# jpinedev/OpenCL-Raytracer

Hardware: AMD Instinct MI355X
Metric: Mrays/s (primary+reflect+shadow) at 4096x4096, 1/2/4/8 GPU; max RGB diff vs ref (higher is better)
Workload: dtype f32

## Files before the change

opencl-raytracer_amd/csrc/rt_device.h:

```cpp
#pragma once

#include <hip/hip_runtime.h>
#include <stdint.h>

namespace rt {

constexpr float kMaxFloat = 3.402823466e+38F;

struct HotObject {
    float4 row0;
    float4 row1;
    float4 row2;
    uint32_t type;
    uint32_t pad[3];
};
struct ColdObject {
    float4 mv_row[4];
    float4 inv_row3;
    float4 amb_absorb;
    float4 dif_shine;
    float4 spec_type;
};
struct ObjectRecord {
    float4 inv_row[3];
// ... 351 lines not shown
    uint32_t line = (p + kWarmAhead) * 2u + (__lane_id() & 63u);
    const uint32_t last = n_pairs * 2u - 1u;
    line = line < last ? line : last;
    w.pending = *reinterpret_cast<const uint32_t*>(reinterpret_cast<const char*>(pairs) + (uint64_t)line * 64u);
}
__device__ __forceinline__ void l2_warm_finish(Warm& w) {
    asm volatile("" ::"v"(w.sink ^ w.pending));
}

template <int AM, bool DW0>
__device__ __forceinline__ void closest_hit(const HotPair* __restrict__ pairs, uint32_t n_pairs, const Ray& ray, float& T,
                                            int& index) {
    if (n_pairs == 0) return;
    const RaySplat r = splat(ray);
    Warm warm;
    HotPair a = pairs[0];
    uint32_t p = 0;
    for (; p + 1 < n_pairs; p += 2) {
        if ((p & (kWarmPeriod - 1u)) == 0u) l2_warm(pairs, n_pairs, p, warm);
        const HotPair b = pairs[p + 1];
        closest_pair<AM, DW0>(a, (int)p, r, T, index);
        a = pairs[(p + 2 < n_pairs) ? p + 2 : p + 1];
        closest_pair<AM, DW0>(b, (int)p + 1, r, T, index);
    }
    if (p < n_pairs) closest_pair<AM, DW0>(a, (int)p, r, T, index);
    l2_warm_finish(warm);
}

template <int AM>
__device__ __forceinline__ bool occludes(uint32_t type, float sx, float sy, float sz, float dx, float dy, float dz) {
    float t;
    bool cand = false;
    if (type == 0u) cand = sphere_candidate<AM>(sx, sy, sz, dx, dy, dz, t);
    else if (type == 1u) cand = box_candidate<AM>(sx, sy, sz, dx, dy, dz, t);
    return cand && !(t >= 1.f);
}

template <int AM>
__device__ __forceinline__ bool any_hit_pair(const HotPair& h, const RaySplat& r) {
    f2 sx, sy, sz, dx, dy, dz;
    pair_object_space<AM, true>(h, r, sx, sy, sz, dx, dy, dz);
    bool occ = false;
    if ((h.type_a | h.type_b) == 0u) {
        const f2 rad = pair_radical<AM>(sx, sy, sz, dx, dy, dz);
        const bool ca = !(rad.x < 0), cb = !(rad.y < 0);
        if (ca || cb) {
            if (ca) occ = occludes<AM>(0u, sx.x, sy.x, sz.x, dx.x, dy.x, dz.x);
            if (cb && !occ) occ = occludes<AM>(0u, sx.y, sy.y, sz.y, dx.y, dy.y, dz.y);
        }
    } else {
        occ = occludes<AM>(h.type_a, sx.x, sy.x, sz.x, dx.x, dy.x, dz.x);
        if (!occ) occ = occludes<AM>(h.type_b, sx.y, sy.y, sz.y, dx.y, dy.y, dz.y);
    }
    return occ;
}

template <int AM>
__device__ __forceinline__ bool any_hit_before_one(const HotPair* __restrict__ pairs, uint32_t n_pairs, const Ray& ray,
                                                   uint32_t* pairs_visited = nullptr) {
    if (pairs_visited) *pairs_visited = 0;
    if (n_pairs == 0) return false;
    const RaySplat r = splat(ray);
    bool occluded = false, done = false;
    Warm warm;
    HotPair a = pairs[0];
    uint32_t p = 0;
    for (; p + 1 < n_pairs; p += 2) {
        if ((p & (kWarmPeriod - 1u)) == 0u) l2_warm(pairs, n_pairs, p, warm);
        const HotPair b = pairs[p + 1];
        occluded |= any_hit_pair<AM>(a, r);
        a = pairs[(p + 2 < n_pairs) ? p + 2 : p + 1];
        occluded |= any_hit_pair<AM>(b, r);
        if (__ballot(!occluded) == 0ull) { done = true; p += 2; break; }
    }
    if (!done && p < n_pairs) {
        if (__ballot(!occluded) != 0ull) { occluded |= any_hit_pair<AM>(a, r); p = n_pairs; }
    }
    if (pairs_visited) *pairs_visited = p;
    l2_warm_finish(warm);
    return occluded;
}

template <int AM, bool DW0>
__device__ __forceinline__ void object_space_one(const RT_CONST HotObjectC* o, const Ray& ray, float& sx, float& sy,
                                                 float& sz, float& dx, float& dy, float& dz) {
    const f4 r0 = o->row0, r1 = o->row1, r2 = o->row2;
    sx = row4<AM>(r0.x, r0.y, r0.z, r0.w, ray.sx, ray.sy, ray.sz, ray.sw);
    sy = row4<AM>(r1.x, r1.y, r1.z, r1.w, ray.sx, ray.sy, ray.sz, ray.sw);
    sz = row4<AM>(r2.x, r2.y, r2.z, r2.w, ray.sx, ray.sy, ray.sz, ray.sw);
    if constexpr (DW0) {
        dx = row3<AM>(r0.x, r0.y, r0.z, ray.dx, ray.dy, ray.dz);
        dy = row3<AM>(r1.x, r1.y, r1.z, ray.dx, ray.dy, ray.dz);
        dz = row3<AM>(r2.x, r2.y, r2.z, ray.dx, ray.dy, ray.dz);
    } else {
        dx = row4<AM>(r0.x, r0.y, r0.z, r0.w, ray.dx, ray.dy, ray.dz, ray.dw);
        dy = row4<AM>(r1.x, r1.y, r1.z, r1.w, ray.dx, ray.dy, ray.dz, ray.dw);
        dz = row4<AM>(r2.x, r2.y, r2.z, r2.w, ray.dx, ray.dy, ray.dz, ray.dw);
    }
}

template <int AM, bool DW0>
__device__ __forceinline__ void closest_hit_small(const HotObject* __restrict__ hot_, uint32_t n, bool use_mask, uint64_t mask,
                                                  const Ray& ray, float& T, int& index) {
    const RT_CONST HotObjectC* hot = (const RT_CONST HotObjectC*)(hot_);
    if (use_mask) {
        while (mask) {
            const int k = __builtin_ctzll(mask);
            mask &= mask - 1ull;
            float sx, sy, sz, dx, dy, dz;
            object_space_one<AM, DW0>(hot + k, ray, sx, sy, sz, dx, dy, dz);
            closest_update<AM>(hot[k].type, sx, sy, sz, dx, dy, dz, k, T, index);
        }
    } else {
        for (uint32_t k = 0; k < n; ++k) {
            float sx, sy, sz, dx, dy, dz;
            object_space_one<AM, DW0>(hot + k, ray, sx, sy, sz, dx, dy, dz);
            closest_update<AM>(hot[k].type, sx, sy, sz, dx, dy, dz, (int)k, T, index);
        }
    }
}

template <int AM>
__device__ __forceinline__ bool any_hit_small(const HotObject* __restrict__ hot_, uint32_t n, const Ray& ray) {
    const RT_CONST HotObjectC* hot = (const RT_CONST HotObjectC*)(hot_);
    bool occluded = false;
    for (uint32_t k = 0; k < n; ++k) {
        float sx, sy, sz, dx, dy, dz;
        object_space_one<AM, true>(hot + k, ray, sx, sy, sz, dx, dy, dz);
        occluded |= occludes<AM>(hot[k].type, sx, sy, sz, dx, dy, dz);
        if (__ballot(!occluded) == 0ull) break;
    }
    return occluded;
}

struct ObjRows {
    float4 r0, r1, r2;
    uint32_t type, pad0;
};

template <int AM>
__device__ __forceinline__ void materialise(const ObjectRecord* __restrict__ objrec, const ColdObject* __restrict__ cold,
                                            int index, float t, const Ray& ray, HitRec& h, bool affine = false, ObjRows* rows = nullptr,
                                            float* absorption = nullptr) {
    const ObjectRecord* o = objrec + index;
    const ColdObject* c = cold + index;
    const uint32_t type = o->type;
    if (rows) { rows->r0 = o->inv_row[0]; rows->r1 = o->inv_row[1]; rows->r2 = o->inv_row[2]; rows->type = type; rows->pad0 = o->pad0; }
    if (absorption) *absorption = o->absorption;
    if (type == 2u) {
        const float4 e1 = o->inv_row[1], e2 = o->inv_row[2];
        h.px = fma_<AM>(t, ray.dx, ray.sx);
        h.py = fma_<AM>(t, ray.dy, ray.sy);
        h.pz = fma_<AM>(t, ray.dz, ray.sz);
        h.pw = fma_<AM>(t, ray.dw, ray.sw);
        float nx = e1.y * e2.z - e1.z * e2.y;
        float ny = e1.z * e2.x - e1.x * e2.z;
        float nz = e1.x * e2.y - e1.y * e2.x;
        normalize3(nx, ny, nz);
        h.nx = nx; h.ny = ny; h.nz = nz;
        const float k2 = dot3(ray.dx, ray.dy, ray.dz, nx, ny, nz) * -2.0f;
        h.rx = fma_<AM>(k2, nx, ray.dx);
        h.ry = fma_<AM>(k2, ny, ray.dy);
        h.rz = fma_<AM>(k2, nz, ray.dz);
        h.index = index;
        return;
    }
    const float4 r0 = o->inv_row[0], r1 = o->inv_row[1], r2 = o->inv_row[2];
    const float sx = row4<AM>(r0.x, r0.y, r0.z, r0.w, ray.sx, ray.sy, ray.sz, ray.sw);
    const float sy = row4<AM>(r1.x, r1.y, r1.z, r1.w, ray.sx, ray.sy, ray.sz, ray.sw);
    const float sz = row4<AM>(r2.x, r2.y, r2.z, r2.w, ray.sx, ray.sy, ray.sz, ray.sw);
    const float dx = row4<AM>(r0.x, r0.y, r0.z, r0.w, ray.dx, ray.dy, ray.dz, ray.dw);
    const float dy = row4<AM>(r1.x, r1.y, r1.z, r1.w, ray.dx, ray.dy, ray.dz, ray.dw);
    const float dz = row4<AM>(r2.x, r2.y, r2.z, r2.w, ray.dx, ray.dy, ray.dz, ray.dw);
    float sw, dw;
    if (affine) {
        sw = ray.sw;
        dw = ray.dw;
    } else {
        const float4 r3 = c->inv_row3;
        sw = row4<AM>(r3.x, r3.y, r3.z, r3.w, ray.sx, ray.sy, ray.sz, ray.sw);
        dw = row4<AM>(r3.x, r3.y, r3.z, r3.w, ray.dx, ray.dy, ray.dz, ray.dw);
// ... 272 lines not shown
```

opencl-raytracer_amd/csrc/rt_wavefront.hip:

```cpp
#include "rt_kernels.h"
#include "rt_grid.h"

#include <algorithm>
#include <cstdio>
#include <cstdlib>
#include <cstring>

namespace rt {

enum : uint32_t {
    F_SX, F_SY, F_SZ, F_SW, F_DX, F_DY, F_DZ, F_DW,
    F_A0, F_A1, F_A2, F_A3, F_A4, F_A5, F_A6, F_A7,
    F_PX, F_PY, F_PZ, F_HIDX,
    F_NX, F_NY, F_NZ, F_PHASE,
    F_ABR, F_ABG, F_ABB, F_AP,
    F_RES_T, F_RES_I, F_RES_ANY, F_BOUNCES,
    F_RX, F_RY, F_RZ, F_PW,
    F_RR, F_RG, F_RB, F_SPARE,
    F_AR, F_AG, F_AB, F_DR, F_DG, F_DB, F_SR, F_SG,
    F_SB, F_CR, F_CG, F_CB,
    F_COUNT
};
static_assert(F_COUNT % 4 == 0 && F_PX == 16, "blocks of four after the two ray records");
enum : uint32_t { PH_DONE = 0, PH_PRIMARY = 1, PH_SHADOW_PRIMARY = 2, PH_SHADOW_REFLECT = 3, PH_REFLECT = 4 };
constexpr uint32_t PH_FLAG_REFLECTION_SENT = 0x100u;
constexpr uint32_t PH_FLAG_REFLECTION_PENDING = 0x200u;
constexpr uint32_t kPhaseLightShift = 10;
static_assert(kPhaseLightShift == 10, "rt_create limits the light count to 2^22 - 1");

enum : uint32_t {
    RS_NEXT_CLOSEST = 0, RS_NEXT_ANY = 1,
    RS_SLICE_A = 2, RS_SLICE_B = 3,
    RS_N_CLOSEST = 4, RS_N_ANY = 5,
    RS_CUR = 6,
    RS_FINISH = 7,
    RS_ROUNDS = 8,
    RS_NEXT_SINGLES = 10,
    RS_N_SINGLES = 11,
    RS_WORDS = 16
};

struct WfParams {
    RenderParams rp;
    float* st;
    uint32_t* qs[2][2];
    uint32_t* q_closest;
    uint32_t* q_any;
    uint32_t* q_prev_closest;
    uint32_t* q_prev_any;
    uint32_t* counts;
    const HotPair* shadow_pairs;
    GridDesc grid;
    ScreenTiles tiles;
    LightTiles ltiles;
    BlockGrid bgrid;
    uint32_t n_prev_closest, n_prev_any;
    int kernel;
    uint32_t first_round;
    uint32_t identity_queue;
    uint32_t count_rays;
};

__device__ __forceinline__ bool resolve_round(WfParams& w) {
    const uint32_t* rs = w.counts;
    const bool odd = (rs[RS_CUR] & 1u) != 0u;
    w.q_prev_closest = odd ? w.qs[1][0] : w.qs[0][0];
    w.q_prev_any = odd ? w.qs[1][1] : w.qs[0][1];
    w.q_closest = odd ? w.qs[0][0] : w.qs[1][0];
    w.q_any = odd ? w.qs[0][1] : w.qs[1][1];
    w.n_prev_closest = rs[RS_N_CLOSEST];
    w.n_prev_any = rs[RS_N_ANY];
    return rs[RS_FINISH] == 0u;
}

__device__ __forceinline__ uint64_t pixel_of(const RenderParams& p, uint64_t t) {
    if (!p.wf_tile_order) return t;
    const uint32_t tt = (uint32_t)t;
    const uint32_t tile = tt >> 6, within = tt & 63u;
    const uint32_t trow = tile / p.bundles_x, tcol = tile - trow * p.bundles_x;
    return (uint64_t)(((trow << 3) + (within >> 3)) * p.width + (tcol << 3) + (within & 7u));
}

__device__ __forceinline__ uint64_t field_at(const WfParams& w, uint32_t f, uint64_t i) {
    return (uint64_t)(f & ~3u) * w.rp.n_local + 4u * i + (f & 3u);
}
__device__ __forceinline__ float& F(const WfParams& w, uint32_t f, uint64_t i) { return w.st[field_at(w, f, i)]; }
// ... 82 lines not shown
    if (want_any) q_any[s_base[1] + s_cnt[1][wave] + (uint32_t)__popcll(ba & below)] = id | any_flag;
}

__device__ __forceinline__ unsigned long long wave_sum64(unsigned long long v) {
#pragma unroll
    for (int off = 32; off > 0; off >>= 1) v += __shfl_xor(v, off, 64);
    return v;
}

__device__ __forceinline__ bool begin_pixel(const WfParams& w, uint64_t i);

__global__ __launch_bounds__(kResumeThreads) void wf_begin(const WfParams wk) {
    WfParams w = wk;
    (void)resolve_round(w);
    const RenderParams& p = w.rp;
    const uint64_t i = (uint64_t)blockIdx.x * kResumeThreads + threadIdx.x;
    bool want = false;
    if (i < p.n_local) want = begin_pixel(w, i);
    block_push(want, false, (uint32_t)i, w.q_closest, w.q_any, w.counts);
}

__device__ __forceinline__ uint64_t global_ray_of(const RenderParams& p, uint64_t i) {
    const uint64_t px = pixel_of(p, i);
    if (p.world <= 1u) return px;
    const uint64_t run = px / p.run_rays;
    return (run * p.world + p.rank) * p.tile_rays + (px - run * p.run_rays);
}
__device__ __forceinline__ Ray primary_ray(const RenderParams& p, uint64_t g) {
    Ray ray;
    if (p.pinhole) {
        const uint32_t gi = (uint32_t)g;
        const uint32_t row = gi / p.width;
        const uint32_t col = gi - row * p.width;
        ray.sx = 0.f; ray.sy = 0.f; ray.sz = 0.f; ray.sw = 1.f;
        ray.dx = (float)col - p.half_w;
        ray.dy = (p.height_f - (float)row) - p.half_h;
        ray.dz = p.z;
        ray.dw = 0.f;
    } else {
        const float4 s = p.rays[2 * g];
        const float4 d = p.rays[2 * g + 1];
        ray.sx = s.x; ray.sy = s.y; ray.sz = s.z; ray.sw = s.w;
        ray.dx = d.x; ray.dy = d.y; ray.dz = d.z; ray.dw = d.w;
    }
    return ray;
}
__device__ __forceinline__ Ray closest_ray(const WfParams& w, uint64_t i, bool primary) {
    return primary ? primary_ray(w.rp, global_ray_of(w.rp, i)) : load_ray(w, i, kSlotClosest);
}

__device__ __forceinline__ bool begin_pixel(const WfParams& w, uint64_t i) {
    const RenderParams& p = w.rp;
    if (global_ray_of(p, i) >= p.n_rays) {
        const uint64_t px = pixel_of(p, i);
        if (w.kernel == 0) reinterpret_cast<float*>(p.out)[px] = kMaxFloat;
        else reinterpret_cast<float4*>(p.out)[px] = make_float4(0.f, 0.f, 0.f, 1.0f);
        if (p.aux_t) p.aux_t[px] = kMaxFloat;
        if (p.aux_index) p.aux_index[px] = -1;
        store_block(w, F_NX, i, make_float4(0.f, 0.f, 0.f, __uint_as_float(PH_DONE)));
        return false;
    }
    store_block(w, F_NX, i, make_float4(0.f, 0.f, 0.f, __uint_as_float(PH_PRIMARY)));
    return true;
}

template <int AM, bool DW0>
__global__ __launch_bounds__(256) void wf_trace_closest(const WfParams wk) {
    WfParams w = wk;
    if (!resolve_round(w)) return;
    const uint32_t t = blockIdx.x * 256u + threadIdx.x;
    if (t >= w.n_prev_closest) return;
    const uint64_t i = w.identity_queue ? t : (w.q_prev_closest[t] & kQueuePixel);
    const Ray ray = closest_ray(w, i, w.first_round != 0u);
    float T = kMaxFloat;
    int idx = -1;
    closest_hit<AM, DW0>(w.rp.scene.pairs, w.rp.scene.n_pairs, ray, T, idx);
    store_closest_result(w, i, T, idx);
    const unsigned long long lanes = (unsigned long long)__popcll(__ballot(true));
    if (w.count_rays && (threadIdx.x & 63u) == 0u)
        atomicAdd(&w.rp.counters->tests, 2ull * w.rp.scene.n_pairs * lanes);
}

template <int AM>
__device__ __forceinline__ void tile_candidate(const RT_CONST HotObjectC* o, int k, const Ray& ray, float& T, int& idx, bool& cur_sphere) {
    const uint32_t type = o->type;
    if (type == 2u) {
        const f4 r0 = o->row0, r1 = o->row1, r2 = o->row2;
        float t;
        if (triangle_candidate(r0.x, r0.y, r0.z, r1.x, r1.y, r1.z, r2.x, r2.y, r2.z, r0.w, r1.w, r2.w, __uint_as_float(o->pad[0]), ray, t))
            closest_take(t, k, false, T, idx, cur_sphere);
        return;
    }
    float sx, sy, sz, dx, dy, dz;
    object_space_one<AM, true>(o, ray, sx, sy, sz, dx, dy, dz);
    closest_update_unordered<AM>(type, sx, sy, sz, dx, dy, dz, k, T, idx, cur_sphere);
}

template <int AM>
__global__ __launch_bounds__(256) void wf_trace_primary_tiles(const WfParams wk) {
    WfParams w = wk;
    if (!resolve_round(w)) return;
    const uint32_t t = blockIdx.x * 256u + threadIdx.x;
    if (t >= w.n_prev_closest) return;
    const RenderParams& p = w.rp;
    const uint64_t i = w.identity_queue ? t : (w.q_prev_closest[t] & kQueuePixel);
    const uint64_t g = global_ray_of(p, i);
    const Ray ray = primary_ray(p, g);
    const uint32_t row = (uint32_t)g / p.width, col = (uint32_t)g - row * p.width;
    const uint32_t tile = (row >> 3) * w.tiles.tiles_x + (col >> w.tiles.col_shift);
    const uint32_t first = __builtin_amdgcn_readfirstlane(tile);
    float T = kMaxFloat;
    int idx = -1;
    uint32_t tested = 0;
    if (__ballot(tile != first) == 0ull) {
        bool cur_sphere = false;
        const RT_CONST HotObjectC* hot = (const RT_CONST HotObjectC*)(p.scene.hot);
        for (uint32_t a = 0; a < w.grid.n_always; ++a) {
            const int k = (int)w.grid.always[a];
            tile_candidate<AM>(hot + k, k, ray, T, idx, cur_sphere);
        }
        for (uint32_t a = 0; a < w.tiles.n_global; ++a) {
            const int k = (int)w.tiles.entries[w.tiles.global_begin + a];
            tile_candidate<AM>(hot + k, k, ray, T, idx, cur_sphere);
        }
        const uint32_t e0 = w.tiles.tile_start[first], e1 = w.tiles.tile_start[first + 1];
        tested = w.grid.n_always + w.tiles.n_global + (e1 - e0);
        for (uint32_t e = e0; e < e1; ++e) {
            const int k = (int)w.tiles.entries[e];
            tile_candidate<AM>(hot + k, k, ray, T, idx, cur_sphere);
        }
    } else {
        closest_hit_grid<AM, true>(w.grid, p.scene.hot, ray, T, idx, tested);
    }
    store_closest_result(w, i, T, idx);
    if (w.count_rays) atomicAdd(&w.rp.counters->tests, (unsigned long long)tested);
}

#ifndef RT_SEGMENT
#define RT_SEGMENT 256
#endif
constexpr uint32_t kSegment = RT_SEGMENT;
#ifndef RT_TICKET_REGIONS
#define RT_TICKET_REGIONS 8
#endif
constexpr uint32_t kTicketRegions = RT_TICKET_REGIONS;
constexpr uint32_t kTicketStride = 16;
constexpr uint32_t kTicketWords = 16u * kTicketStride;
constexpr uint32_t kTicketBase = 16;

#ifndef RT_WALK_DEDUPE
#define RT_WALK_DEDUPE 1
#endif
#ifndef RT_REFILL_MIN
#define RT_REFILL_MIN 16
#endif
#ifndef RT_SKIP_CAP
#define RT_SKIP_CAP 2
#endif
#ifndef RT_INLINE_LAST_SHADOW
#define RT_INLINE_LAST_SHADOW 1
#endif
#ifndef RT_FLAT_PARK
#define RT_FLAT_PARK 1
#endif
#ifndef RT_CELL_INLINE
#define RT_CELL_INLINE 1
#endif
#ifndef RT_SKIP_FEW_LANES
#define RT_SKIP_FEW_LANES 12
#endif
#ifndef RT_WALK_FIRST_CELL
#define RT_WALK_FIRST_CELL 0
#endif
#ifndef RT_DEFER_PENDING
#define RT_DEFER_PENDING 8
#endif
#ifndef RT_DEFER_STUCK_SHIFT
#define RT_DEFER_STUCK_SHIFT 2
#endif

__device__ __forceinline__ bool misses_bounding_sphere2(const float4 s, float sx, float sy, float sz, float dx, float dy, float dz,
                                                        float dd, float alpha) {
    const float ox = s.x - sx, oy = s.y - sy, oz = s.z - sz;
    const float oo = __builtin_fmaf(oz, oz, __builtin_fmaf(oy, oy, ox * ox));
    const float od = __builtin_fmaf(oz, dz, __builtin_fmaf(oy, dy, ox * dx));
    const float c = oo - s.w;
    const float disc = __builtin_fmaf(od, od, -(dd * __builtin_fmaf(-alpha, oo, c)));
    return disc < 0.f || (od < 0.f && c > 1.0e-5f * oo);
}

__device__ __forceinline__ void lt_block_entry(const LightTiles& lt, uint32_t lo, uint32_t hi, float4& sphere, float& key) {
    const float r = (float)((hi >> 16) & 0xffu) * lt.rstep;
    sphere = make_float4(__builtin_fmaf((float)(lo & 0xffffu), lt.lat_step, lt.lat_lox), __builtin_fmaf((float)(lo >> 16), lt.lat_step, lt.lat_loy),
                         __builtin_fmaf((float)(hi & 0xffffu), lt.lat_step, lt.lat_loz), r * r);
    key = (float)(hi >> 24) * lt.kstep;
}

struct RunCursor {
    uint32_t seg, n_runs, next, seg_end, region, regions_tried;
    bool dynamic;
    __device__ __forceinline__ bool grab(uint32_t n_queue, uint32_t* __restrict__ run_ctr, uint32_t lane) {
        for (;;) {
            const uint32_t lo = (uint32_t)(((uint64_t)n_runs * region) / kTicketRegions);
            const uint32_t hi = (uint32_t)(((uint64_t)n_runs * (region + 1u)) / kTicketRegions);
            uint32_t r = 0;
            if (lane == 0u) r = atomicAdd(run_ctr + region * kTicketStride, 1u);
            r = __builtin_amdgcn_readfirstlane(r) + lo;
            if (r < hi) {
                next = r * seg;
                seg_end = (n_queue - next < seg) ? n_queue : next + seg;
                return true;
            }
            if (++regions_tried >= kTicketRegions) return false;
            region = (region + 1u == kTicketRegions) ? 0u : region + 1u;
        }
    }
// ... 1273 lines not shown
        const float wgt = 1.f - ap;
        if (am != kUnfused) { abr = fma_<kFused>(wgt, rr, abr); abg = fma_<kFused>(wgt, rg, abg); abb = fma_<kFused>(wgt, rb, abb); }
        else { abr = fma_<kUnfused>(wgt, rr, abr); abg = fma_<kUnfused>(wgt, rg, abg); abb = fma_<kUnfused>(wgt, rb, abb); }
    }
    write_pixel<2>(c, abr, abg, abb);
}

__device__ __forceinline__ void store_loop_state(Ctx& c, float abr, float abg, float abb, float rr, float rg, float rb, float ap,
                                                 uint32_t bounces, bool keep_reflect_color) {
    const uint64_t i = c.i;
    store_block(c.w, F_ABR, i, make_float4(abr, abg, abb, ap));
    U(c.w, F_BOUNCES, i) = bounces;
    if (keep_reflect_color) store_block(c.w, F_RR, i, make_float4(rr, rg, rb, 0.f));
}

template <int AM>
__device__ __forceinline__ void loop_step(Ctx& c, const HitRec& from, float abr, float abg, float abb, float rr, float rg,
                                          float rb, float ap, uint32_t bounces) {
    const Scene& S = c.w.rp.scene;
    const uint32_t before = bounces;
    bounces = bounces - 1u;
    if (!(before > 0u)) { finish_reflect(c, AM, abr, abg, abb, rr, rg, rb, ap, bounces); return; }
    c.reference += 1;
    const bool absorbing = (ap <= 0.999f);
    if (!absorbing && !S.literal) { finish_reflect(c, AM, abr, abg, abb, rr, rg, rb, ap, bounces); return; }
    if (c.flags & PH_FLAG_REFLECTION_SENT) {
        const uint64_t i = c.i;
        float T;
        int idx;
        Ray ray;
        if (c.pre) {
            T = c.pre_res.x;
            idx = (int)__float_as_uint(c.pre_res.y);
            ray = c.pre_ray0;
            patch_nan_result(c.w, ray, T, idx);
        } else {
            closest_result(c.w, i, false, T, idx);
        }
        if (T == kMaxFloat) { finish_reflect(c, AM, abr, abg, abb, rr, rg, rb, ap, bounces); return; }
        if (!c.pre) ray = load_ray(c.w, i, kSlotClosest);
        ray.dw = 0.0f;
        HitRec rh;
        ObjRows rows;
        float absorb_rh;
        materialise<AM>(S.objrec, S.cold, idx, T, ray, rh, S.affine != 0u, &rows, &absorb_rh);
        store_loop_state(c, abr, abg, abb, rr, rg, rb, ap, bounces, false);
        if (c.pre) {
            c.pre_acc = make_float4(abr, abg, abb, ap);
            c.pre_res.w = __uint_as_float(bounces);
        }
        const float ra = (1.f - ap) * absorb_rh;
        begin_shade_lit<2, AM>(c, rh, false, bounces, ap + ra, rows);
        return;
    }
    Ray ray;
    reflection_ray<AM>(from, ray);
    ray.dw = __uint_as_float(0xffffffffu);
    store_ray(c.w, c.i, ray, kSlotClosest);
    store_loop_state(c, abr, abg, abb, rr, rg, rb, ap, bounces, true);
    U(c.w, F_PHASE, c.i) = PH_REFLECT;
    c.want_closest = true;
    c.traced += 1;
}

template <int KERNEL, int AM>
__device__ __forceinline__ void shade_done(Ctx& c, const HitRec& h, bool primary, float cr, float cg, float cb) {
    const Scene& S = c.w.rp.scene;
    if (KERNEL == 1) { write_pixel<1>(c, cr, cg, cb); return; }
    const uint64_t i = c.i;
    if (primary) {
        const float ap = S.cold[h.index].amb_absorb.w;
        loop_step<AM>(c, h, cr * ap, cg * ap, cb * ap, 0.f, 0.f, 0.f, ap, c.w.rp.max_bounces);
    } else {
        const float4 acc = c.pre ? c.pre_acc : load_block(c.w, F_ABR, i);
        float ap = acc.w;
        float abr = acc.x, abg = acc.y, abb = acc.z;
        const float ra = (1.f - ap) * S.cold[h.index].amb_absorb.w;
        abr = fma_<AM>(ra, cr, abr); abg = fma_<AM>(ra, cg, abg); abb = fma_<AM>(ra, cb, abb);
        ap = ap + ra;
        loop_step<AM>(c, h, abr, abg, abb, cr, cg, cb, ap, c.pre ? __float_as_uint(c.pre_res.w) : U(c.w, F_BOUNCES, i));
    }
}

template <int KERNEL, int AM>
__device__ __forceinline__ void resume_pixel(Ctx& c) {
    const WfParams& w = c.w;
    const uint64_t i = c.i;
    const Scene& S = w.rp.scene;
    c.pre = false;
    c.nblock = w.identity_queue ? make_float4(0.f, 0.f, 0.f, __uint_as_float(PH_PRIMARY)) : load_block(w, F_NX, i);
    const uint32_t word = __float_as_uint(c.nblock.w);
    const uint32_t phase = word & 0xffu;
    c.flags = word & (PH_FLAG_REFLECTION_SENT | PH_FLAG_REFLECTION_PENDING);
    c.li = word >> kPhaseLightShift;
    if (phase == PH_PRIMARY) {
        float T;
        int idx;
        closest_result(w, i, true, T, idx);
        const bool hit = (KERNEL == 2) ? !(T == kMaxFloat) : (T < kMaxFloat);
        c.traced += 1; c.reference += 1; c.hits += hit ? 1 : 0;
        if (w.rp.aux_t) w.rp.aux_t[pixel_of(w.rp, i)] = T;
        if (w.rp.aux_index) w.rp.aux_index[pixel_of(w.rp, i)] = hit ? idx : -1;
        if (KERNEL == 0) {
            reinterpret_cast<float*>(w.rp.out)[pixel_of(w.rp, i)] = hit ? T : kMaxFloat;
            U(w, F_PHASE, i) = PH_DONE;
        } else if (!hit) {
            write_pixel<KERNEL>(c, 0.f, 0.f, 0.f);
        } else {
            const Ray ray = closest_ray(w, i, true);
            HitRec h;
            ObjRows rows;
            float absorb_h;
            materialise<AM>(S.objrec, S.cold, idx, T, ray, h, S.affine != 0u, &rows, &absorb_h);
            begin_shade<KERNEL, AM>(c, h, true, w.rp.max_bounces, absorb_h, rows);
        }
    } else if (phase == PH_SHADOW_PRIMARY || phase == PH_SHADOW_REFLECT) {
        c.pre = true;
        c.pre_hit = load_block(w, F_PX, i);
        c.pre_res = load_block(w, F_RES_T, i);
        c.pre_acc = load_block(w, F_ABR, i);
        c.pre_ray0 = load_ray(w, i, kSlotClosest);
        resume_shadow<KERNEL, AM>(c, phase == PH_SHADOW_PRIMARY);
    } else if (phase == PH_REFLECT) {
        float T;
        int idx;
        closest_result(w, i, false, T, idx);
        const float4 acc = load_block(w, F_ABR, i), rc = load_block(w, F_RR, i);
        const float ap = acc.w;
        const uint32_t bounces = U(w, F_BOUNCES, i);
        const float abr = acc.x, abg = acc.y, abb = acc.z;
        const float rr = rc.x, rg = rc.y, rb = rc.z;
        if (T == kMaxFloat || !(ap <= 0.999f)) {
            finish_reflect(c, AM, abr, abg, abb, rr, rg, rb, ap, bounces);
        } else {
            Ray ray = load_ray(w, i, kSlotClosest);
            ray.dw = 0.0f;
            HitRec rh;
            ObjRows rows;
            float absorb_rh;
            materialise<AM>(S.objrec, S.cold, idx, T, ray, rh, S.affine != 0u, &rows, &absorb_rh);
            begin_shade<KERNEL, AM>(c, rh, false, bounces, ap + (1.f - ap) * absorb_rh, rows);
        }
    }
}

__device__ __forceinline__ bool duplicate_entry(const WfParams& w, uint32_t t, uint32_t entry) {
    return (t < w.n_prev_closest) && (entry & kQueueAlsoShadow) != 0u;
}

__device__ __forceinline__ void add_ray_counters(const WfParams& w, const Ctx& c) {
    const unsigned long long a = wave_sum64(c.traced), b = wave_sum64(c.reference), h = wave_sum64(c.hits), t = wave_sum64(c.tests);
    if ((threadIdx.x & 63u) == 0u && (a | b | h | t)) {
        atomicAdd(&w.rp.counters->traced, a);
        atomicAdd(&w.rp.counters->reference, b);
        atomicAdd(&w.rp.counters->hits, h);
        if (t) atomicAdd(&w.rp.counters->tests, t);
    }
}

#ifndef RT_RESUME_WAVES_PER_EU
#define RT_RESUME_WAVES_PER_EU 4
#endif
template <int KERNEL, int AM>
__global__ __launch_bounds__(kResumeThreads) __attribute__((amdgpu_waves_per_eu(RT_RESUME_WAVES_PER_EU))) void wf_resume(const WfParams wk) {
    WfParams w = wk;
    if (!resolve_round(w)) return;
    if (blockIdx.x * kResumeThreads >= w.n_prev_closest + w.n_prev_any) return;
    if (w.counts[RS_N_SINGLES] == 0u && (blockIdx.x + 1u) * kResumeThreads <= w.n_prev_closest) return;
    const uint32_t t = blockIdx.x * kResumeThreads + threadIdx.x;
    const uint32_t total = w.n_prev_closest + w.n_prev_any;
    Ctx c{w, 0, 0ull, 0ull, 0ull, false, false, 0u, 0u, make_float4(0.f, 0.f, 0.f, 0.f), false, {}, {}, {}, {}};
    if (t < total) {
        const uint32_t entry = w.identity_queue ? t : ((t < w.n_prev_closest) ? w.q_prev_closest[t] : w.q_prev_any[t - w.n_prev_closest]);
        c.i = entry & kQueuePixel;
        if (!duplicate_entry(w, t, entry)) resume_pixel<KERNEL, AM>(c);
    }
    block_push(c.want_closest, c.want_any, (uint32_t)c.i, w.q_closest, w.q_any, w.counts, c.any_flag);
    if (w.count_rays) add_ray_counters(w, c);
}

template <int KERNEL, int AM>
__global__ __launch_bounds__(256) void wf_finish(const WfParams wk) {
    WfParams w = wk;
    (void)resolve_round(w);
    if (w.counts[RS_FINISH] != 1u) return;
    const uint32_t t = blockIdx.x * 256u + threadIdx.x;
    const uint32_t total = w.n_prev_closest + w.n_prev_any;
    Ctx c{w, 0, 0ull, 0ull, 0ull, false, false, 0u, 0u, make_float4(0.f, 0.f, 0.f, 0.f), false, {}, {}, {}, {}};
    uint32_t tested = 0;
    if (t < total) {
        const uint32_t entry = (t < w.n_prev_closest) ? w.q_prev_closest[t] : w.q_prev_any[t - w.n_prev_closest];
        c.i = entry & kQueuePixel;
        if (!duplicate_entry(w, t, entry)) {
            bool do_closest = (t < w.n_prev_closest) || (U(w, F_PHASE, c.i) & PH_FLAG_REFLECTION_PENDING) != 0u;
            bool do_any = !(t < w.n_prev_closest);
            for (;;) {
                if (do_any) {
                    uint32_t li;
                    Ray ray;
                    if (shadow_rays_rebuilt(w)) {
                        ray = shadow_of_pixel<AM>(w, c.i, false, li);
                    } else {
                        ray = load_ray(w, c.i, kSlotShadow);
                        li = __float_as_uint(ray.dw);
                    }
                    bool blocked;
                    if (w.ltiles.enabled && li == w.ltiles.light) {
                        blocked = last_light_blocked<AM>(w, ray, tested);
                    } else {
                        bool walked = false;
                        blocked = false;
                        if (w.bgrid.enabled && w.grid.n_always == 0u) {
                            Ray r1 = ray;
                            r1.sw = 1.0f; r1.dw = 0.0f;
                            blocked = any_hit_blocks<AM>(w.bgrid, w.grid, w.rp.scene.hot, r1, walked, tested);
                        }
                        if (!walked) blocked = any_hit_grid<AM>(w.grid, w.rp.scene, ray, tested);
                    }
                    U(w, F_RES_ANY, c.i) = blocked ? 0u : 1u;
                }
                if (do_closest) {
                    Ray ray = load_ray(w, c.i, kSlotClosest);
                    float T = kMaxFloat;
                    int idx = -1;
                    bool walked = false;
                    if (w.bgrid.enabled && w.grid.n_always == 0u) {
                        const uint32_t note = __float_as_uint(ray.dw);
                        ray.sw = 1.0f; ray.dw = 0.0f;
                        walked = closest_hit_blocks<AM>(w.bgrid, w.grid, w.rp.scene.hot, ray, note, T, idx, tested);
                    }
                    if (!walked) closest_hit_grid<AM, true>(w.grid, w.rp.scene.hot, ray, T, idx, tested);
                    store_closest_result(w, c.i, T, idx);
                }
                c.want_closest = false;
                c.want_any = false;
                resume_pixel<KERNEL, AM>(c);
                if (!c.want_closest && !c.want_any) break;
                do_closest = c.want_closest;
                do_any = c.want_any;
            }
        }
    }
    if (w.count_rays) {
        add_ray_counters(w, c);
        if (tested) atomicAdd(&w.rp.counters->tests, (unsigned long long)tested);
    }
}

constexpr uint32_t kMinSlicePairs = 2048;
constexpr uint32_t kMaxSlices = 16;

__global__ __launch_bounds__(256) void wf_advance(uint32_t* __restrict__ rs, uint32_t finish_threshold, uint32_t allow_finish) {
    for (uint32_t k = threadIdx.x; k < 2u * kTicketWords; k += 256u) rs[kTicketBase + k] = 0u;
    if (threadIdx.x != 0u) return;
    if (rs[RS_FINISH] != 0u) return;
    const uint32_t nc = rs[RS_NEXT_CLOSEST], na = rs[RS_NEXT_ANY];
    rs[RS_N_CLOSEST] = nc;
    rs[RS_N_ANY] = na;
// ... 27 lines not shown
    uint64_t waves = (n + 63) / 64;
    if (waves > max_waves) waves = max_waves;
    if (waves == 0) waves = 1;
    return dim3((uint32_t)((waves + 3u) / 4u));
}

size_t wavefront_state_bytes(uint64_t n_local) { return (size_t)F_COUNT * sizeof(float) * (size_t)n_local; }
size_t wavefront_queue_bytes(uint64_t n_local) { return sizeof(uint32_t) * (size_t)n_local; }
size_t wavefront_counter_bytes() { return sizeof(uint32_t) * (size_t)(kTicketBase + 2u * kTicketWords); }

template <int AM, bool ANY>
static void launch_persistent(const WfParams& w, uint64_t n_max, uint32_t* ticket, hipStream_t s, bool shared) {
    const bool mesh = w.grid.has_triangles != 0u;
    uint64_t any_cap = std::min<uint64_t>(RT_MAX_WAVES_ANY_SHARED, n_max <= (3ull << 20) ? 2048u : (mesh ? 4096u : 2560u));
    uint64_t closest_cap = shared ? (n_max <= (3ull << 20) ? std::min<uint64_t>(RT_MAX_WAVES_CLOSEST_SHARED, 4096u) : (mesh ? RT_MAX_WAVES : RT_MAX_WAVES_CLOSEST_SHARED)) : RT_MAX_WAVES;
    if (const char* env = std::getenv("RT_WAVES_CLOSEST")) closest_cap = (uint64_t)std::max(64, std::atoi(env));
    if (const char* env = std::getenv("RT_WAVES_ANY")) any_cap = (uint64_t)std::max(64, std::atoi(env));
    const dim3 grid = persistent_grid(n_max, ANY ? any_cap : closest_cap), block(256);
    const bool tri = w.grid.has_triangles != 0u;
    const char* walk2_env = std::getenv("RT_WALK2");
    const char* walk3_env = std::getenv("RT_WALK3");
    if (!ANY && w.bgrid.enabled && !(walk3_env && walk3_env[0] == '0')) {
        if (tri) {
            if (w.count_rays) hipLaunchKernelGGL((wf_walk_blocks<AM, true, true>), grid, block, 0, s, w, ticket);
            else hipLaunchKernelGGL((wf_walk_blocks<AM, false, true>), grid, block, 0, s, w, ticket);
        } else {
            if (w.count_rays) hipLaunchKernelGGL((wf_walk_blocks<AM, true, false>), grid, block, 0, s, w, ticket);
            else hipLaunchKernelGGL((wf_walk_blocks<AM, false, false>), grid, block, 0, s, w, ticket);
        }
        return;
    }
    const bool walk2_allowed = !walk2_env || (ANY ? std::strcmp(walk2_env, "any") == 0 : std::strcmp(walk2_env, "closest") == 0) || std::strcmp(walk2_env, "both") == 0;
    if (!tri && w.grid.walk_rec && walk2_allowed && (!ANY || !w.ltiles.enabled || w.ltiles.walk_base != 0u || w.ltiles.blocks_enabled)) {
        if (w.count_rays) hipLaunchKernelGGL((wf_walk<AM, ANY, true>), grid, block, 0, s, w, ticket);
        else hipLaunchKernelGGL((wf_walk<AM, ANY, false>), grid, block, 0, s, w, ticket);
        return;
    }
    if (w.count_rays) {
        if (tri) hipLaunchKernelGGL((wf_trace_grid_persistent<AM, ANY, true, true>), grid, block, 0, s, w, ticket);
        else hipLaunchKernelGGL((wf_trace_grid_persistent<AM, ANY, true, false>), grid, block, 0, s, w, ticket);
    } else {
        if (tri) hipLaunchKernelGGL((wf_trace_grid_persistent<AM, ANY, false, true>), grid, block, 0, s, w, ticket);
        else hipLaunchKernelGGL((wf_trace_grid_persistent<AM, ANY, false, false>), grid, block, 0, s, w, ticket);
    }
}

template <int KERNEL, int AM>
static hipError_t run_wavefront(WfParams w, WavefrontBuffers& buf, hipStream_t stream, uint32_t* rounds_out) {
    hipError_t e;
    const uint64_t n = w.rp.n_local;
    w.st = buf.state;
    w.counts = buf.counts;
    w.shadow_pairs = buf.shadow_pairs;
    w.grid = buf.grid;
    w.tiles = buf.tiles;
    w.ltiles = buf.light_tiles;
    w.bgrid = buf.blocks;
    for (int a = 0; a < 2; ++a) { w.qs[a][0] = buf.q_closest[a]; w.qs[a][1] = buf.q_any[a]; }
    uint32_t* rs = buf.counts;
    if ((e = hipMemsetAsync(rs, 0, wavefront_counter_bytes(), stream)) != hipSuccess) return e;
    uint64_t finish_threshold = std::max<uint64_t>(2048, n / 128);
    if (const char* env = std::getenv("RT_WF_FINISH_THRESHOLD")) finish_threshold = (uint64_t)std::atoll(env);
    if (finish_threshold > 0xffffffffull) finish_threshold = 0xffffffffull;
    const bool use_grid = w.grid.enabled && !w.rp.scene.literal;
    const uint64_t last_run = n ? (n - 1u) / w.rp.run_rays : 0u;
    const bool padded = w.rp.world > 1u && n > 0u && (last_run * w.rp.world + w.rp.rank) * w.rp.tile_rays + (n - last_run * w.rp.run_rays) > w.rp.n_rays;
    static const bool always_begin = std::getenv("RT_WF_ALWAYS_BEGIN") != nullptr;
    const bool identity = !padded && !always_begin && n > 0;
    if (identity) {
        hipLaunchKernelGGL(wf_identity_round, dim3(1), dim3(1), 0, stream, rs, (uint32_t)n);
        if ((e = hipGetLastError()) != hipSuccess) return e;
    } else {
        hipLaunchKernelGGL(wf_begin, dim3((uint32_t)((n + kResumeThreads - 1) / kResumeThreads)), dim3(kResumeThreads), 0, stream, w);
        if ((e = hipGetLastError()) != hipSuccess) return e;
        hipLaunchKernelGGL(wf_advance, dim3(1), dim3(256), 0, stream, rs, (uint32_t)finish_threshold, 0u);
        if ((e = hipGetLastError()) != hipSuccess) return e;
    }

    static const bool one_stream = std::getenv("RT_WF_ONE_STREAM") != nullptr;
    auto enqueue_round = [&](bool first, uint64_t nc_max, uint64_t na_max) -> hipError_t {
        hipError_t e2;
        w.first_round = first ? 1u : 0u;
        w.identity_queue = (first && identity) ? 1u : 0u;
        const bool side_by_side = use_grid && nc_max && na_max && buf.side_stream && !one_stream;
        hipStream_t any_stream = stream;
        if (side_by_side) {
            any_stream = buf.side_stream;
            if ((e2 = hipEventRecord(buf.ev_fork, stream)) != hipSuccess) return e2;
            if ((e2 = hipStreamWaitEvent(any_stream, buf.ev_fork, 0)) != hipSuccess) return e2;
            launch_persistent<AM, true>(w, na_max, rs + kTicketBase + kTicketWords, any_stream, true);
            if ((e2 = hipGetLastError()) != hipSuccess) return e2;
            if ((e2 = hipEventRecord(buf.ev_join, any_stream)) != hipSuccess) return e2;
        }
        if (nc_max) {
            if (use_grid && first && w.tiles.enabled && w.rp.pinhole) {
                hipLaunchKernelGGL((wf_trace_primary_tiles<AM>), grid_for(nc_max), dim3(256), 0, stream, w);
            } else if (use_grid) {
                launch_persistent<AM, false>(w, nc_max, rs + kTicketBase, stream, side_by_side);
            } else {
                if (first && !w.rp.dir_w_zero) hipLaunchKernelGGL((wf_trace_closest<AM, false>), grid_for(nc_max), dim3(256), 0, stream, w);
                else hipLaunchKernelGGL((wf_trace_closest<AM, true>), grid_for(nc_max), dim3(256), 0, stream, w);
            }
            if ((e2 = hipGetLastError()) != hipSuccess) return e2;
        }
        if (side_by_side) {
            if ((e2 = hipStreamWaitEvent(stream, buf.ev_join, 0)) != hipSuccess) return e2;
        } else if (na_max) {
            if (w.rp.scene.literal) {
                hipLaunchKernelGGL((wf_trace_any_literal<AM>), grid_for(na_max), dim3(256), 0, stream, w);
                if ((e2 = hipGetLastError()) != hipSuccess) return e2;
            } else if (use_grid) {
                launch_persistent<AM, true>(w, na_max, rs + kTicketBase + kTicketWords, stream, false);
                if ((e2 = hipGetLastError()) != hipSuccess) return e2;
            } else {
                const uint32_t n_pairs = w.rp.scene.n_pairs;
                uint32_t n_slices = n_pairs / kMinSlicePairs;
                n_slices = n_slices < 1u ? 1u : (n_slices > kMaxSlices ? kMaxSlices : n_slices);
                for (uint32_t sl = 0; sl < n_slices; ++sl) {
                    const uint32_t lo = (uint32_t)((uint64_t)n_pairs * sl / n_slices);
                    const uint32_t hi = (uint32_t)((uint64_t)n_pairs * (sl + 1) / n_slices);
                    const bool last = (sl + 1 == n_slices);
                    uint32_t* q_out = last ? nullptr : buf.q_slice[sl & 1u];
                    uint32_t* n_out = rs + (sl & 1u ? RS_SLICE_B : RS_SLICE_A);
                    const uint32_t* q_in = sl ? buf.q_slice[(sl - 1u) & 1u] : nullptr;
                    const uint32_t* n_in = rs + ((sl - 1u) & 1u ? RS_SLICE_B : RS_SLICE_A);
                    if (!last && (e2 = hipMemsetAsync(n_out, 0, sizeof(uint32_t), stream)) != hipSuccess) return e2;
                    hipLaunchKernelGGL((wf_trace_any_slice<AM>), grid_for(na_max), dim3(256), 0, stream, w, q_in, n_in, lo, hi,
                                       q_out, n_out, sl == 0 ? 1u : 0u);
                    if ((e2 = hipGetLastError()) != hipSuccess) return e2;
                }
            }
        }
        const uint64_t total_max = nc_max + na_max;
        hipLaunchKernelGGL((wf_resume<KERNEL, AM>), dim3((uint32_t)((total_max + kResumeThreads - 1) / kResumeThreads)),
                           dim3(kResumeThreads), 0, stream, w);
        if ((e2 = hipGetLastError()) != hipSuccess) return e2;
        hipLaunchKernelGGL(wf_advance, dim3(1), dim3(256), 0, stream, rs, (uint32_t)finish_threshold, use_grid ? 1u : 0u);
        return hipGetLastError();
    };

    uint32_t batch = 1;
    if (KERNEL == 1) batch = w.rp.scene.n_lights + 1u;
    else if (KERNEL == 2) batch = w.rp.scene.literal ? 8u : w.rp.max_bounces + 2u;
    if (batch > 12u) batch = 12u;
    if (const char* env = std::getenv("RT_WF_BATCH")) batch = (uint32_t)std::max(1, std::atoi(env));
    bool first = true;
    uint64_t nc_max = n, na_max = 0;
    for (;;) {
        for (uint32_t r = 0; r < batch; ++r) {
            if ((e = enqueue_round(first, nc_max, na_max)) != hipSuccess) return e;
            if (first) { first = false; nc_max = (KERNEL == 0) ? 0 : n; na_max = (KERNEL == 0) ? 0 : n; }
            if (nc_max + na_max == 0) break;
        }
        if (use_grid) {
            w.first_round = 0u;
            w.identity_queue = 0u;
            hipLaunchKernelGGL((wf_finish<KERNEL, AM>), grid_for(finish_threshold ? finish_threshold : 1), dim3(256), 0, stream, w);
            if ((e = hipGetLastError()) != hipSuccess) return e;
        }
        if ((e = hipMemcpyAsync(buf.h_counts, rs, RS_WORDS * sizeof(uint32_t), hipMemcpyDeviceToHost, stream)) != hipSuccess) return e;
        if ((e = hipStreamSynchronize(stream)) != hipSuccess) return e;
        if (std::getenv("RT_ROUND_STATS"))
            std::fprintf(stderr, "[rounds] after %u round(s): closest queue %u, shadow queue %u, hand-over %u\n", buf.h_counts[RS_ROUNDS],
                         buf.h_counts[RS_N_CLOSEST], buf.h_counts[RS_N_ANY], buf.h_counts[RS_FINISH]);
        if (buf.h_counts[RS_FINISH] != 0u) break;
        if (nc_max + na_max == 0) break;
        const uint64_t alive = (uint64_t)buf.h_counts[RS_N_CLOSEST] + buf.h_counts[RS_N_ANY];
        nc_max = std::min<uint64_t>(n, alive);
        na_max = std::min<uint64_t>(n, alive);
        batch = std::getenv("RT_ROUND_STATS") ? 1u : 8u;
    }
    if (rounds_out) *rounds_out = buf.h_counts[RS_ROUNDS];
    return hipSuccess;
}

template <int KERNEL>
static hipError_t run_wavefront_arith(const WfParams& w, int arith, WavefrontBuffers& buf, hipStream_t stream, uint32_t* rounds_out) {
    switch (arith) {
        case kUnfused: return run_wavefront<KERNEL, kUnfused>(w, buf, stream, rounds_out);
        case kFused: return run_wavefront<KERNEL, kFused>(w, buf, stream, rounds_out);
        case kDeviceCL: return run_wavefront<KERNEL, kDeviceCL>(w, buf, stream, rounds_out);
        default: return hipErrorInvalidValue;
    }
}

hipError_t launch_wavefront(const RenderParams& p, int kernel, int arith, bool count, WavefrontBuffers& buf,
                            hipStream_t stream, uint32_t* rounds_out) {
    if (p.n_local >= 0x7fffffffull) return hipErrorInvalidValue;
    WfParams w;
    std::memset(&w, 0, sizeof(w));
    w.rp = p;
    w.kernel = kernel;
    w.count_rays = count ? 1u : 0u;
    switch (kernel) {
        case 0: return run_wavefront_arith<0>(w, arith, buf, stream, rounds_out);
        case 1: return run_wavefront_arith<1>(w, arith, buf, stream, rounds_out);
        case 2: return run_wavefront_arith<2>(w, arith, buf, stream, rounds_out);
        default: return hipErrorInvalidValue;
    }
}

}
```

Measured before the change: 9678.

## Fuse primary tile tracing with primary shading and prefetch tile records

Adds a fused kernel for the first wavefront round that traces primary rays against screen tiles and then runs the primary shading step in the same thread. This skips storing and reloading the closest-hit result and drops the separate resume launch. Tile candidate lists are also software-pipelined: the next object id and hot record are loaded with volatile vector loads while the current candidate is tested. The fused kernel uses the resume kernel's launch bounds and waves-per-EU limit, which may raise register pressure or lower occupancy for the tracing part. It can be turned off with an environment variable.

```diff
diff --git a/opencl-raytracer_amd/csrc/rt_device.h b/opencl-raytracer_amd/csrc/rt_device.h
--- a/opencl-raytracer_amd/csrc/rt_device.h
+++ b/opencl-raytracer_amd/csrc/rt_device.h
@@ -457,9 +457,8 @@
 }
 
 template <int AM, bool DW0>
-__device__ __forceinline__ void object_space_one(const RT_CONST HotObjectC* o, const Ray& ray, float& sx, float& sy,
-                                                 float& sz, float& dx, float& dy, float& dz) {
-    const f4 r0 = o->row0, r1 = o->row1, r2 = o->row2;
+__device__ __forceinline__ void object_space_rows(const f4 r0, const f4 r1, const f4 r2, const Ray& ray, float& sx, float& sy,
+                                                  float& sz, float& dx, float& dy, float& dz) {
     sx = row4<AM>(r0.x, r0.y, r0.z, r0.w, ray.sx, ray.sy, ray.sz, ray.sw);
     sy = row4<AM>(r1.x, r1.y, r1.z, r1.w, ray.sx, ray.sy, ray.sz, ray.sw);
     sz = row4<AM>(r2.x, r2.y, r2.z, r2.w, ray.sx, ray.sy, ray.sz, ray.sw);
@@ -472,6 +471,11 @@
         dy = row4<AM>(r1.x, r1.y, r1.z, r1.w, ray.dx, ray.dy, ray.dz, ray.dw);
         dz = row4<AM>(r2.x, r2.y, r2.z, r2.w, ray.dx, ray.dy, ray.dz, ray.dw);
     }
+}
+template <int AM, bool DW0>
+__device__ __forceinline__ void object_space_one(const RT_CONST HotObjectC* o, const Ray& ray, float& sx, float& sy,
+                                                 float& sz, float& dx, float& dy, float& dz) {
+    object_space_rows<AM, DW0>(o->row0, o->row1, o->row2, ray, sx, sy, sz, dx, dy, dz);
 }
 
 template <int AM, bool DW0>
diff --git a/opencl-raytracer_amd/csrc/rt_wavefront.hip b/opencl-raytracer_amd/csrc/rt_wavefront.hip
--- a/opencl-raytracer_amd/csrc/rt_wavefront.hip
+++ b/opencl-raytracer_amd/csrc/rt_wavefront.hip
@@ -2,6 +2,7 @@
 #include "rt_grid.h"
 
 #include <algorithm>
+#include <cstddef>
 #include <cstdio>
 #include <cstdlib>
 #include <cstring>
@@ -250,18 +251,78 @@
 }
 
 template <int AM>
-__device__ __forceinline__ void tile_candidate(const RT_CONST HotObjectC* o, int k, const Ray& ray, float& T, int& idx, bool& cur_sphere) {
-    const uint32_t type = o->type;
+__device__ __forceinline__ void tile_candidate(const HotObjectC& o, int k, const Ray& ray, float& T, int& idx, bool& cur_sphere) {
+    const uint32_t type = o.type;
     if (type == 2u) {
-        const f4 r0 = o->row0, r1 = o->row1, r2 = o->row2;
+        const f4 r0 = o.row0, r1 = o.row1, r2 = o.row2;
         float t;
-        if (triangle_candidate(r0.x, r0.y, r0.z, r1.x, r1.y, r1.z, r2.x, r2.y, r2.z, r0.w, r1.w, r2.w, __uint_as_float(o->pad[0]), ray, t))
+        if (triangle_candidate(r0.x, r0.y, r0.z, r1.x, r1.y, r1.z, r2.x, r2.y, r2.z, r0.w, r1.w, r2.w, __uint_as_float(o.pad[0]), ray, t))
             closest_take(t, k, false, T, idx, cur_sphere);
         return;
     }
     float sx, sy, sz, dx, dy, dz;
-    object_space_one<AM, true>(o, ray, sx, sy, sz, dx, dy, dz);
+    object_space_rows<AM, true>(o.row0, o.row1, o.row2, ray, sx, sy, sz, dx, dy, dz);
     closest_update_unordered<AM>(type, sx, sy, sz, dx, dy, dz, k, T, idx, cur_sphere);
+}
+
+typedef uint32_t u32x8 __attribute__((ext_vector_type(8)));
+typedef uint32_t u32x4 __attribute__((ext_vector_type(4)));
+typedef uint32_t u32x2 __attribute__((ext_vector_type(2)));
+__device__ __forceinline__ HotObjectC load_hot_record(const RT_CONST HotObjectC* o) {
+    const u32x8 a = *(const volatile RT_CONST u32x8*)o;
+    const u32x4 b = *(const volatile RT_CONST u32x4*)((const RT_CONST char*)o + 32);
+    const u32x2 c = *(const volatile RT_CONST u32x2*)((const RT_CONST char*)o + 48);
+    HotObjectC r;
+    r.row0 = f4{__uint_as_float(a[0]), __uint_as_float(a[1]), __uint_as_float(a[2]), __uint_as_float(a[3])};
+    r.row1 = f4{__uint_as_float(a[4]), __uint_as_float(a[5]), __uint_as_float(a[6]), __uint_as_float(a[7])};
+    r.row2 = f4{__uint_as_float(b[0]), __uint_as_float(b[1]), __uint_as_float(b[2]), __uint_as_float(b[3])};
+    r.type = c[0];
+    r.pad[0] = c[1]; r.pad[1] = 0u; r.pad[2] = 0u;
+    return r;
+}
+static_assert(offsetof(HotObjectC, row2) == 32 && offsetof(HotObjectC, type) == 48 && offsetof(HotObjectC, pad) == 52, "load_hot_record");
+__device__ __forceinline__ int load_list_id(const RT_CONST uint32_t* p) { return (int)*(const volatile RT_CONST uint32_t*)p; }
+template <int AM>
+__device__ __forceinline__ void tile_list(const RT_CONST HotObjectC* hot, const RT_CONST uint32_t* ids, uint32_t e0, uint32_t e1,
+                                          const Ray& ray, float& T, int& idx, bool& cur_sphere) {
+    if (e0 >= e1) return;
+    const uint32_t last = e1 - 1u;
+    int k = load_list_id(ids + e0);
+    int k_next = load_list_id(ids + (e0 < last ? e0 + 1u : last));
+    HotObjectC rec = load_hot_record(hot + k);
+    for (uint32_t e = e0; e < e1; ++e) {
+        const int k_after = load_list_id(ids + (e + 2u < e1 ? e + 2u : last));
+        const HotObjectC rec_next = load_hot_record(hot + k_next);
+        tile_candidate<AM>(rec, k, ray, T, idx, cur_sphere);
+        rec = rec_next;
+        k = k_next;
+        k_next = k_after;
+    }
+}
+
+template <int AM>
+__device__ __forceinline__ void trace_primary_tile(const WfParams& w, uint64_t i, Ray& ray, float& T, int& idx, uint32_t& tested) {
+    const RenderParams& p = w.rp;
+    const uint64_t g = global_ray_of(p, i);
+    ray = primary_ray(p, g);
+    const uint32_t row = (uint32_t)g / p.width, col = (uint32_t)g - row * p.width;
+    const uint32_t tile = (row >> 3) * w.tiles.tiles_x + (col >> w.tiles.col_shift);
+    const uint32_t first = __builtin_amdgcn_readfirstlane(tile);
+    T = kMaxFloat;
+    idx = -1;
+    tested = 0;
+    if (__ballot(tile != first) == 0ull) {
+        bool cur_sphere = false;
+        const RT_CONST HotObjectC* hot = (const RT_CONST HotObjectC*)(p.scene.hot);
+        const RT_CONST uint32_t* entries = (const RT_CONST uint32_t*)(w.tiles.entries);
+        tile_list<AM>(hot, (const RT_CONST uint32_t*)(w.grid.always), 0u, w.grid.n_always, ray, T, idx, cur_sphere);
+        tile_list<AM>(hot, entries, w.tiles.global_begin, w.tiles.global_begin + w.tiles.n_global, ray, T, idx, cur_sphere);
+        const uint32_t e0 = w.tiles.tile_start[first], e1 = w.tiles.tile_start[first + 1];
+        tested = w.grid.n_always + w.tiles.n_global + (e1 - e0);
+        tile_list<AM>(hot, entries, e0, e1, ray, T, idx, cur_sphere);
+    } else {
+        closest_hit_grid<AM, true>(w.grid, p.scene.hot, ray, T, idx, tested);
+    }
 }
 
 template <int AM>
@@ -270,36 +331,12 @@
     if (!resolve_round(w)) return;
     const uint32_t t = blockIdx.x * 256u + threadIdx.x;
     if (t >= w.n_prev_closest) return;
-    const RenderParams& p = w.rp;
     const uint64_t i = w.identity_queue ? t : (w.q_prev_closest[t] & kQueuePixel);
-    const uint64_t g = global_ray_of(p, i);
-    const Ray ray = primary_ray(p, g);
-    const uint32_t row = (uint32_t)g / p.width, col = (uint32_t)g - row * p.width;
-    const uint32_t tile = (row >> 3) * w.tiles.tiles_x + (col >> w.tiles.col_shift);
-    const uint32_t first = __builtin_amdgcn_readfirstlane(tile);
-    float T = kMaxFloat;
-    int idx = -1;
-    uint32_t tested = 0;
-    if (__ballot(tile != first) == 0ull) {
-        bool cur_sphere = false;
-        const RT_CONST HotObjectC* hot = (const RT_CONST HotObjectC*)(p.scene.hot);
-        for (uint32_t a = 0; a < w.grid.n_always; ++a) {
-            const int k = (int)w.grid.always[a];
-            tile_candidate<AM>(hot + k, k, ray, T, idx, cur_sphere);
-        }
-        for (uint32_t a = 0; a < w.tiles.n_global; ++a) {
-            const int k = (int)w.tiles.entries[w.tiles.global_begin + a];
-            tile_candidate<AM>(hot + k, k, ray, T, idx, cur_sphere);
-        }
-        const uint32_t e0 = w.tiles.tile_start[first], e1 = w.tiles.tile_start[first + 1];
-        tested = w.grid.n_always + w.tiles.n_global + (e1 - e0);
-        for (uint32_t e = e0; e < e1; ++e) {
-            const int k = (int)w.tiles.entries[e];
-            tile_candidate<AM>(hot + k, k, ray, T, idx, cur_sphere);
-        }
-    } else {
-        closest_hit_grid<AM, true>(w.grid, p.scene.hot, ray, T, idx, tested);
-    }
+    Ray ray;
+    float T;
+    int idx;
+    uint32_t tested;
+    trace_primary_tile<AM>(w, i, ray, T, idx, tested);
     store_closest_result(w, i, T, idx);
     if (w.count_rays) atomicAdd(&w.rp.counters->tests, (unsigned long long)tested);
 }
@@ -1739,6 +1776,30 @@
     }
 }
 
+template <int KERNEL, int AM, bool RAY_GIVEN>
+__device__ __forceinline__ void primary_step(Ctx& c, float T, int idx, const Ray& given) {
+    const WfParams& w = c.w;
+    const uint64_t i = c.i;
+    const Scene& S = w.rp.scene;
+    const bool hit = (KERNEL == 2) ? !(T == kMaxFloat) : (T < kMaxFloat);
+    c.traced += 1; c.reference += 1; c.hits += hit ? 1 : 0;
+    if (w.rp.aux_t) w.rp.aux_t[pixel_of(w.rp, i)] = T;
+    if (w.rp.aux_index) w.rp.aux_index[pixel_of(w.rp, i)] = hit ? idx : -1;
+    if (KERNEL == 0) {
+        reinterpret_cast<float*>(w.rp.out)[pixel_of(w.rp, i)] = hit ? T : kMaxFloat;
+        U(w, F_PHASE, i) = PH_DONE;
+    } else if (!hit) {
+        write_pixel<KERNEL>(c, 0.f, 0.f, 0.f);
+    } else {
+        const Ray ray = RAY_GIVEN ? given : closest_ray(w, i, true);
+        HitRec h;
+        ObjRows rows;
+        float absorb_h;
+        materialise<AM>(S.objrec, S.cold, idx, T, ray, h, S.affine != 0u, &rows, &absorb_h);
+        begin_shade<KERNEL, AM>(c, h, true, w.rp.max_bounces, absorb_h, rows);
+    }
+}
+
 template <int KERNEL, int AM>
 __device__ __forceinline__ void resume_pixel(Ctx& c) {
     const WfParams& w = c.w;
@@ -1754,23 +1815,7 @@
         float T;
         int idx;
         closest_result(w, i, true, T, idx);
-        const bool hit = (KERNEL == 2) ? !(T == kMaxFloat) : (T < kMaxFloat);
-        c.traced += 1; c.reference += 1; c.hits += hit ? 1 : 0;
-        if (w.rp.aux_t) w.rp.aux_t[pixel_of(w.rp, i)] = T;
-        if (w.rp.aux_index) w.rp.aux_index[pixel_of(w.rp, i)] = hit ? idx : -1;
-        if (KERNEL == 0) {
-            reinterpret_cast<float*>(w.rp.out)[pixel_of(w.rp, i)] = hit ? T : kMaxFloat;
-            U(w, F_PHASE, i) = PH_DONE;
-        } else if (!hit) {
-            write_pixel<KERNEL>(c, 0.f, 0.f, 0.f);
-        } else {
-            const Ray ray = closest_ray(w, i, true);
-            HitRec h;
-            ObjRows rows;
-            float absorb_h;
-            materialise<AM>(S.objrec, S.cold, idx, T, ray, h, S.affine != 0u, &rows, &absorb_h);
-            begin_shade<KERNEL, AM>(c, h, true, w.rp.max_bounces, absorb_h, rows);
-        }
+        primary_step<KERNEL, AM, false>(c, T, idx, Ray{});
     } else if (phase == PH_SHADOW_PRIMARY || phase == PH_SHADOW_REFLECT) {
         c.pre = true;
         c.pre_hit = load_block(w, F_PX, i);
@@ -1831,6 +1876,27 @@
         const uint32_t entry = w.identity_queue ? t : ((t < w.n_prev_closest) ? w.q_prev_closest[t] : w.q_prev_any[t - w.n_prev_closest]);
         c.i = entry & kQueuePixel;
         if (!duplicate_entry(w, t, entry)) resume_pixel<KERNEL, AM>(c);
+    }
+    block_push(c.want_closest, c.want_any, (uint32_t)c.i, w.q_closest, w.q_any, w.counts, c.any_flag);
+    if (w.count_rays) add_ray_counters(w, c);
+}
+
+template <int KERNEL, int AM>
+__global__ __launch_bounds__(kResumeThreads) __attribute__((amdgpu_waves_per_eu(RT_RESUME_WAVES_PER_EU))) void wf_primary(const WfParams wk) {
+    WfParams w = wk;
+    if (!resolve_round(w)) return;
+    if (blockIdx.x * kResumeThreads >= w.n_prev_closest) return;
+    const uint32_t t = blockIdx.x * kResumeThreads + threadIdx.x;
+    Ctx c{w, t, 0ull, 0ull, 0ull, false, false, 0u, 0u, make_float4(0.f, 0.f, 0.f, __uint_as_float(PH_PRIMARY)), false, {}, {}, {}, {}};
+    if (t < w.n_prev_closest) {
+        Ray ray;
+        float T;
+        int idx;
+        uint32_t tested;
+        trace_primary_tile<AM>(w, c.i, ray, T, idx, tested);
+        patch_nan_result(w, ray, T, idx);
+        c.tests = tested;
+        primary_step<KERNEL, AM, true>(c, T, idx, ray);
     }
     block_push(c.want_closest, c.want_any, (uint32_t)c.i, w.q_closest, w.q_any, w.counts, c.any_flag);
     if (w.count_rays) add_ray_counters(w, c);
@@ -2024,6 +2090,8 @@
         hipError_t e2;
         w.first_round = first ? 1u : 0u;
         w.identity_queue = (first && identity) ? 1u : 0u;
+        const char* fused_env = std::getenv("RT_PRIMARY_FUSED");
+        const bool fused_primary = use_grid && first && identity && nc_max && w.tiles.enabled && w.rp.pinhole && !(fused_env && fused_env[0] == '0');
         const bool side_by_side = use_grid && nc_max && na_max && buf.side_stream && !one_stream;
         hipStream_t any_stream = stream;
         if (side_by_side) {
@@ -2035,7 +2103,10 @@
             if ((e2 = hipEventRecord(buf.ev_join, any_stream)) != hipSuccess) return e2;
         }
         if (nc_max) {
-            if (use_grid && first && w.tiles.enabled && w.rp.pinhole) {
+            if (fused_primary) {
+                hipLaunchKernelGGL((wf_primary<KERNEL, AM>), dim3((uint32_t)((nc_max + kResumeThreads - 1) / kResumeThreads)),
+                                   dim3(kResumeThreads), 0, stream, w);
+            } else if (use_grid && first && w.tiles.enabled && w.rp.pinhole) {
                 hipLaunchKernelGGL((wf_trace_primary_tiles<AM>), grid_for(nc_max), dim3(256), 0, stream, w);
             } else if (use_grid) {
                 launch_persistent<AM, false>(w, nc_max, rs + kTicketBase, stream, side_by_side);
@@ -2073,10 +2144,12 @@
                 }
             }
         }
-        const uint64_t total_max = nc_max + na_max;
-        hipLaunchKernelGGL((wf_resume<KERNEL, AM>), dim3((uint32_t)((total_max + kResumeThreads - 1) / kResumeThreads)),
-                           dim3(kResumeThreads), 0, stream, w);
-        if ((e2 = hipGetLastError()) != hipSuccess) return e2;
+        if (!fused_primary) {
+            const uint64_t total_max = nc_max + na_max;
+            hipLaunchKernelGGL((wf_resume<KERNEL, AM>), dim3((uint32_t)((total_max + kResumeThreads - 1) / kResumeThreads)),
+                               dim3(kResumeThreads), 0, stream, w);
+            if ((e2 = hipGetLastError()) != hipSuccess) return e2;
+        }
         hipLaunchKernelGGL(wf_advance, dim3(1), dim3(256), 0, stream, rs, (uint32_t)finish_threshold, use_grid ? 1u : 0u);
         return hipGetLastError();
     };
```

Result: no change. 9735, median of 6 (+0.6%).
